# leejaehot/GaussianGrasper

Hardware: AMD Instinct MI355X
Metric: rendered views/sec (fwd+bwd) at 1M Gaussians, 1600x1200, 32-ch feature (higher is better)
Workload: dtype f32; 1 GPU; BASELINE config 4 per-GPU share: 1000000 Gaussians, 1600x1200, SH deg 4 rgb + 32-ch feature + depth + normal images per view (nerfstudio plugin route: the timed callable is FusedGaussianSplattingModel.get_outputs(camera) of gaussiangrasper_amd.plugin (the class train.sh loads, on stub.py's stand-ins for nerfstudio's base model and Cameras) — one fused rasterize operator per view), fwd+bwd, 8 views; route=plugin, deterministic_backward=False, python_gc=gc.freeze() after the warm-up (bench.freeze_gc), view_pipeline=backward of view k beside forward of view k + 1 on two streams, num_gaussians=1000000, feature_dim=32, n_visible=992125, parallelism=view-parallel x1, replicated Gaussians, grad_allreduce_bytes=472000000, grad_allreduce=per parameter, overlapped with the last view's backward

## Files before the change

### gaussiangrasper_amd/csrc/binning.hip

```cpp
#include "scan.h"

__device__ __forceinline__ int64_t dev_count(int64_t n, const int64_t *__restrict__ n_dev) {
    if (n_dev) {
        const int64_t d = *n_dev;
        if (d < n) n = d;
    }
    return n;
}

#define RS_THREADS 256
#define RS_WAVES (RS_THREADS / GG_WAVE)
#ifndef GG_RS_BIG
#define GG_RS_BIG 16
#endif
static inline int rs_items(int64_t n) { return n >= (int64_t)4096 * 1024 ? GG_RS_BIG : 4; }

__global__ __launch_bounds__(256) void count_kernel(int N, const int32_t *__restrict__ nth,
                                                    unsigned long long *__restrict__ out) {
    __shared__ unsigned long long part[4];
    unsigned long long acc = 0;
    for (int i = blockIdx.x * blockDim.x + threadIdx.x; i < N; i += gridDim.x * blockDim.x)
        acc += (unsigned long long)(uint32_t)nth[i];
    for (int off = 32; off > 0; off >>= 1) acc += __shfl_down(acc, off, 64);
    if ((threadIdx.x & 63) == 0) part[threadIdx.x >> 6] = acc;
// ... 127 lines not shown
        int64_t idx = wbase + (int64_t)it * GG_WAVE + lane;
        bool valid = idx < n;
        uint32_t d = (key[it] >> shift) & mask;
        uint64_t peers = __ballot(valid);
#pragma unroll
        for (int b = 0; b < 8; ++b) {
            if (b < nbits) {
                bool bit = (d >> b) & 1u;
                uint64_t m = __ballot(bit);
                peers &= bit ? m : ~m;
            }
        }
        uint32_t cnt = (uint32_t)__popcll(peers);
        uint32_t before = (uint32_t)__popcll(peers & lt_mask);
        uint32_t old = 0u;
        if (valid && before == 0) old = atomicAdd(&whist[wave][d], cnt);
        old = __shfl(old, (int)__builtin_ctzll(peers | (1ull << 63)), 64);
        rank[it] = old + before;
    }
    __syncthreads();
    __shared__ uint32_t lstart[256];
    __shared__ uint32_t skey[RS_TILE], sval[RS_TILE];
    {
        uint32_t run = 0;
        for (int w = 0; w < RS_WAVES; ++w) {
            uint32_t c = whist[w][tid];
            whist[w][tid] = run;
            run += c;
        }
        uint32_t incl = run;
        for (int off = 1; off < 64; off <<= 1) {
            uint32_t u = __shfl_up(incl, off, 64);
            if (lane >= off) incl += u;
        }
        if (lane == 63) wsum[wave] = incl;
        __syncthreads();
        uint32_t wpre = 0;
        for (int w = 0; w < wave; ++w) wpre += wsum[w];
        lstart[tid] = wpre + incl - run;
    }
    __syncthreads();
#pragma unroll
    for (int it = 0; it < RS_ITEMS; ++it) {
        int64_t idx = wbase + (int64_t)it * GG_WAVE + lane;
        if (idx < n) {
            uint32_t d = (key[it] >> shift) & mask;
            uint32_t lp = lstart[d] + whist[wave][d] + rank[it];
            skey[lp] = key[it];
            sval[lp] = val[it];
        }
    }
    __syncthreads();
    const int64_t left = n - (int64_t)blockIdx.x * RS_TILE;
    const int count = (int)(left < RS_TILE ? left : RS_TILE);
    for (int jj = tid; jj < count; jj += RS_THREADS) {
        const uint32_t k = skey[jj];
        const uint32_t d = (k >> shift) & mask;
        const uint32_t dst = digit_base[d] + ((uint32_t)jj - lstart[d]);
        keys_out[dst] = k;
        vals_out[dst] = sval[jj];
    }
}


typedef unsigned long long u64;
#define DB_BLOCKS 64
#define DB_THREADS 1024
#define DB_CAP 512
#define DB_MAX_BUCKETS 32768
static inline int db_buckets(int N) {
    int nb = 256;
    while (nb < DB_MAX_BUCKETS && nb * 64 < N) nb <<= 1;
    return nb;
}
struct DbRange {
    uint32_t kmin;
    u64 mul;
};
struct DbParts {
    const uint32_t *lo, *hi;
    int n;
};
__device__ __forceinline__ DbRange db_range_of(const DbParts mm, int nb, uint32_t *s_mm ) {
    const int tid = threadIdx.x;
    if (tid < 64) {
        uint32_t lo = 0xFFFFFFFFu, hi = 0u;
        for (int i = tid; i < mm.n; i += 64) {
            lo = min(lo, mm.lo[i]);
            hi = max(hi, mm.hi[i]);
        }
        for (int off = 32; off > 0; off >>= 1) {
            lo = min(lo, (uint32_t)__shfl_xor((int)lo, off, 64));
            hi = max(hi, (uint32_t)__shfl_xor((int)hi, off, 64));
        }
        if (tid == 0) { s_mm[0] = lo; s_mm[1] = hi; }
    }
    __syncthreads();
    DbRange r;
    const uint32_t lo = s_mm[0], hi = s_mm[1];
    r.kmin = lo;
    const u64 span = hi >= lo ? (u64)(hi - lo) + 1ull : 1ull;
    r.mul = (((u64)nb) << 32) / span;
    return r;
}
__device__ __forceinline__ uint32_t db_bucket(const DbRange r, uint32_t key, int nb) {
    if (key == 0xFFFFFFFFu) return (uint32_t)nb;
    return min((uint32_t)(((u64)(key - r.kmin) * r.mul) >> 32), (uint32_t)(nb - 1));
}
__global__ __launch_bounds__(256) void db_range_kernel(int N, DepthSrc dsrc, uint32_t *__restrict__ mm) {
    __shared__ uint32_t s_lo[4], s_hi[4];
    uint32_t lo = 0xFFFFFFFFu, hi = 0u;
    const int stride = 256 * gridDim.x;
    for (int i = blockIdx.x * 256 + threadIdx.x; i < N; i += 4 * stride) {
        uint32_t k[4];
#pragma unroll
        for (int u = 0; u < 4; ++u) k[u] = (i + u * stride < N) ? depth_key(dsrc, i + u * stride) : 0xFFFFFFFFu;
#pragma unroll
        for (int u = 0; u < 4; ++u)
            if (k[u] != 0xFFFFFFFFu) { lo = min(lo, k[u]); hi = max(hi, k[u]); }
    }
    for (int off = 32; off > 0; off >>= 1) {
        lo = min(lo, (uint32_t)__shfl_xor((int)lo, off, 64));
        hi = max(hi, (uint32_t)__shfl_xor((int)hi, off, 64));
    }
    if ((threadIdx.x & 63) == 0) { s_lo[threadIdx.x >> 6] = lo; s_hi[threadIdx.x >> 6] = hi; }
    __syncthreads();
    if (threadIdx.x == 0) {
        mm[blockIdx.x] = min(min(s_lo[0], s_lo[1]), min(s_lo[2], s_lo[3]));
        mm[gridDim.x + blockIdx.x] = max(max(s_hi[0], s_hi[1]), max(s_hi[2], s_hi[3]));
    }
}
#define DB_BOX_MAX 1023
struct DbGeom {
    const float *xys;
    int tiles_x, tiles_y;
};
__device__ __forceinline__ void db_box(const DbGeom g, const DepthSrc d, int i, uint32_t &cnt, uint32_t &box) {
    const int rad = d.radii[i];
    cnt = 0u;
    box = 1u << 20;
    if (rad > 0) {
        int x0, y0, x1, y1;
        gg_tile_bbox(g.xys[2 * (size_t)i], g.xys[2 * (size_t)i + 1], (float)rad, g.tiles_x, g.tiles_y, x0, y0, x1, y1);
        const int bw = x1 - x0;
        if (bw > 0 && y1 > y0) {
            cnt = (uint32_t)(bw * (y1 - y0));
            box = (uint32_t)x0 | ((uint32_t)y0 << 10) | ((uint32_t)bw << 20);
        }
    }
}
template <bool SCATTER>
__global__ __launch_bounds__(DB_THREADS) void db_walk_kernel(int N, int nb, DepthSrc dsrc, DbGeom geom,
                                                             const DbParts mm, uint32_t *__restrict__ G,
                                                             const uint32_t *__restrict__ start, uint4 *__restrict__ recs,
                                                             int32_t *__restrict__ zero = nullptr, int nzero = 0) {
    for (int i = blockIdx.x * DB_THREADS + threadIdx.x; i < nzero; i += DB_BLOCKS * DB_THREADS) zero[i] = 0;
    extern __shared__ uint32_t s_hist[];
    uint32_t *s_mm = s_hist + nb + 1;
    const DbRange r = db_range_of(mm, nb, s_mm);
    const int per = (N + DB_BLOCKS - 1) / DB_BLOCKS;
    const int lo = blockIdx.x * per, hi = min(N, lo + per);
    uint32_t *row = G + (size_t)blockIdx.x * (nb + 1);
    for (int b = threadIdx.x; b <= nb; b += DB_THREADS) s_hist[b] = SCATTER ? start[b] + row[b] : 0u;
    __syncthreads();
    for (int i = lo + threadIdx.x; i < hi; i += 4 * DB_THREADS) {
        uint32_t k[4], cnt[4], box[4];
#pragma unroll
        for (int u = 0; u < 4; ++u) {
            const int iu = i + u * DB_THREADS;
            k[u] = iu < hi ? depth_key(dsrc, iu) : 0u;
            cnt[u] = box[u] = 0u;
            if (SCATTER && iu < hi) db_box(geom, dsrc, iu, cnt[u], box[u]);
        }
#pragma unroll
        for (int u = 0; u < 4; ++u) {
            if (i + u * DB_THREADS < hi) {
                const uint32_t pos = atomicAdd(&s_hist[db_bucket(r, k[u], nb)], 1u);
                if (SCATTER && k[u] != 0xFFFFFFFFu)
                    recs[pos] = make_uint4(k[u], (uint32_t)(i + u * DB_THREADS), cnt[u], box[u]);
            }
        }
    }
    if (!SCATTER) {
        __syncthreads();
        for (int b = threadIdx.x; b <= nb; b += DB_THREADS) row[b] = s_hist[b];
    }
}
__global__ __launch_bounds__(256) void db_prefix_kernel(int nb, uint32_t *__restrict__ G, uint32_t *__restrict__ total) {
    const int b = blockIdx.x * 256 + threadIdx.x;
    if (b > nb) return;
    uint32_t run = 0;
    uint32_t c[DB_BLOCKS];
#pragma unroll
    for (int k = 0; k < DB_BLOCKS; ++k) c[k] = G[(size_t)k * (nb + 1) + b];
#pragma unroll
    for (int k = 0; k < DB_BLOCKS; ++k) {
        G[(size_t)k * (nb + 1) + b] = run;
        run += c[k];
    }
    total[b] = run;
}
__global__ __launch_bounds__(1024) void db_scan_kernel(int n, uint32_t *__restrict__ v) {
    __shared__ uint32_t s_w[2][16];
    const int tid = threadIdx.x, lane = tid & 63, wave = tid >> 6;
    uint32_t carry = 0u;
    int round = 0;
    for (int base = 0; base < n; base += 4 * 4096) {
        uint32_t x[4][4];
#pragma unroll
        for (int q = 0; q < 4; ++q)
#pragma unroll
            for (int k = 0; k < 4; ++k) {
                const int i = base + 4096 * q + 4 * tid + k;
                x[q][k] = i < n ? v[i] : 0u;
            }
#pragma unroll
        for (int q = 0; q < 4; ++q, ++round) {
            if (base + 4096 * q >= n) break;
            const uint32_t mine = x[q][0] + x[q][1] + x[q][2] + x[q][3];
            uint32_t incl = mine;
#pragma unroll
            for (int off = 1; off < 64; off <<= 1) {
                const uint32_t t = __shfl_up(incl, off, 64);
                if (lane >= off) incl += t;
            }
            uint32_t *sw = s_w[round & 1];
            if (lane == 63) sw[wave] = incl;
            __syncthreads();
            uint32_t ex = carry + incl - mine, all = 0u;
#pragma unroll
            for (int w = 0; w < 16; ++w) {
                const uint32_t t = sw[w];
                if (w < wave) ex += t;
                all += t;
            }
            carry += all;
#pragma unroll
            for (int k = 0; k < 4; ++k) {
                const int i = base + 4096 * q + 4 * tid + k;
                if (i < n) v[i] = ex;
                ex += x[q][k];
            }
        }
    }
    if (tid == 0) v[n] = carry;
}

__device__ __forceinline__ void db_ce(u64 &a, u64 &b) {
    const bool sw = b < a;
    const u64 lo = sw ? b : a, hi = sw ? a : b;
    a = lo;
    b = hi;
}
__device__ __forceinline__ void db_bitonic64(u64 *buf, const int n) {
    constexpr int NB = 8, LNB = 3, THREADS = 64;
    const int tid = threadIdx.x & 63;
    int P = NB;
    while (P < n) P <<= 1;
    const u64 INF = ~0ull;
    for (int blk = tid; blk * NB < n; blk += THREADS) {
        u64 v[NB];
#pragma unroll
        for (int r = 0; r < NB; ++r) v[r] = (NB * blk + r < n) ? buf[NB * blk + r] : INF;
#pragma unroll
        for (int k = 2; k <= NB; k <<= 1) {
#pragma unroll
            for (int i = 0; i < NB / 2; ++i) {
                const int b2 = i / (k / 2), off = i % (k / 2);
                db_ce(v[b2 * k + off], v[b2 * k + k - 1 - off]);
            }
#pragma unroll
            for (int j = k >> 2; j >= 1; j >>= 1)
#pragma unroll
                for (int i = 0; i < NB / 2; ++i) {
                    const int lo = ((i & ~(j - 1)) << 1) | (i & (j - 1));
                    db_ce(v[lo], v[lo + j]);
                }
        }
#pragma unroll
        for (int r = 0; r < NB; ++r)
            if (NB * blk + r < n) buf[NB * blk + r] = v[r];
    }
    { __builtin_amdgcn_fence(__ATOMIC_ACQ_REL, "workgroup"); __builtin_amdgcn_wave_barrier(); }
    for (int k = 2 * NB, lk = LNB + 1; k <= P; k <<= 1, ++lk) {
        const int hk = k >> 1;
        for (int i = tid; i < (P >> 1); i += THREADS) {
            const int blk = i >> (lk - 1), off = i & (hk - 1);
            const int lo = blk * k + off, hi = blk * k + k - 1 - off;
            if (hi < n) {
                const u64 a = buf[lo], b = buf[hi];
                if (b < a) { buf[lo] = b; buf[hi] = a; }
            }
        }
        { __builtin_amdgcn_fence(__ATOMIC_ACQ_REL, "workgroup"); __builtin_amdgcn_wave_barrier(); }
        for (int j = k >> 2; j >= NB; j >>= 1) {
            for (int i = tid; i < (P >> 1); i += THREADS) {
                const int lo = ((i & ~(j - 1)) << 1) | (i & (j - 1)), hi = lo + j;
                if (hi < n) {
                    const u64 a = buf[lo], b = buf[hi];
                    if (b < a) { buf[lo] = b; buf[hi] = a; }
                }
            }
            { __builtin_amdgcn_fence(__ATOMIC_ACQ_REL, "workgroup"); __builtin_amdgcn_wave_barrier(); }
        }
        for (int blk = tid; blk * NB < n; blk += THREADS) {
            u64 v[NB];
#pragma unroll
            for (int r = 0; r < NB; ++r) v[r] = (NB * blk + r < n) ? buf[NB * blk + r] : INF;
#pragma unroll
// ... 90 lines not shown
            gid[r] = in ? xw[64 * r + lane] : 0u;
            cntv[r] = in ? xw[DB_RANK_CAP + 64 * r + lane] : 0u;
            boxv[r] = in ? xw[2 * DB_RANK_CAP + 64 * r + lane] : 0u;
        }
    } else if (n <= DB_CAP) {
#define DB_LIM(nv) int nv = n - lane; asm volatile("" : "+v"(nv))
        u64 key[DB_ITEMS];
        {
            DB_LIM(nv);
#pragma unroll
            for (int r = 0; r < DB_ITEMS; ++r) {
                const uint4 rc = (64 * r < nv) ? recs[s0 + 64 * r + lane] : make_uint4(~0u, ~0u, 0u, 0u);
                key[r] = ((u64)rc.x << 32) | rc.y;
            }
        }
        auto pass = [&](const int shift) {
#pragma unroll
            for (int k = 0; k < 4; ++k) hist[lane + 64 * k] = 0u;
            db_wsync();
            {
                DB_LIM(nv);
#pragma unroll
                for (int r = 0; r < DB_ITEMS; ++r)
                    if (64 * r < nv) atomicAdd(&hist[(uint32_t)(key[r] >> shift) & 255u], 1u);
            }
            db_wsync();
            uint32_t tot[4], mine = 0;
            bool constant = false;
#pragma unroll
            for (int k = 0; k < 4; ++k) {
                tot[k] = hist[4 * lane + k];
                constant = constant || tot[k] == (uint32_t)n;
                mine += tot[k];
            }
            if (__ballot(constant) != 0ull) {
                db_wsync();
                return;
            }
            uint32_t incl = mine;
#pragma unroll
            for (int off = 1; off < 64; off <<= 1) {
                const uint32_t u = __shfl_up(incl, off, 64);
                if (lane >= off) incl += u;
            }
            uint32_t ex = incl - mine;
#pragma unroll
            for (int k = 0; k < 4; ++k) {
                hist[4 * lane + k] = ex;
                ex += tot[k];
            }
            db_wsync();
            volatile uint32_t *wh = hist;
            DB_LIM(nv_s);
#pragma unroll
            for (int r = 0; r < DB_ITEMS; ++r) {
                if (64 * r < n) {
                    const bool valid = 64 * r < nv_s;
                    const uint32_t d = (uint32_t)(key[r] >> shift) & 255u;
                    uint64_t peers = __ballot(valid);
#pragma unroll
                    for (int bit = 0; bit < 8; ++bit) {
                        const bool on = (d >> bit) & 1u;
                        const uint64_t m = __ballot(on);
                        peers &= on ? m : ~m;
                    }
                    const uint32_t cnt = (uint32_t)__popcll(peers);
                    const uint32_t before = (uint32_t)__popcll(peers & lt_mask);
                    if (valid && before == 0) wh[d] = wh[d] + cnt;
                    db_wsync();
                    if (valid) buf[wh[d] - cnt + before] = key[r];
                    db_wsync();
                    __builtin_amdgcn_sched_barrier(0);
                }
            }
            {
                DB_LIM(nv);
#pragma unroll
                for (int r = 0; r < DB_ITEMS; ++r) key[r] = (64 * r < nv) ? buf[64 * r + lane] : ~0ull;
            }
            db_wsync();
        };
#pragma nounroll
        for (int round = 0; round < 2; ++round) {
#pragma nounroll
            for (int pb = round == 0 ? 4 : 0; pb < 8; ++pb) pass(8 * pb);
            if (round == 1) break;
            {
                DB_LIM(nv);
#pragma unroll
                for (int r = 0; r < DB_ITEMS; ++r)
                    if (64 * r < nv) buf[64 * r + lane] = key[r];
            }
            db_wsync();
            bool bad = false;
            {
                DB_LIM(nv);
#pragma unroll
                for (int r = 0; r < DB_ITEMS; ++r)
                    if (64 * r + 1 < nv) {
                        const u64 nx = buf[64 * r + lane + 1];
                        bad = bad || ((uint32_t)(nx >> 32) == (uint32_t)(key[r] >> 32) && (uint32_t)nx < (uint32_t)key[r]);
                    }
            }
            db_wsync();
            if (__ballot(bad) == 0ull) break;
        }
#undef DB_LIM
#pragma unroll
        for (int r = 0; r < DB_ITEMS; ++r) gid[r] = (uint32_t)key[r];
    } else {
        for (int i = lane; i < n; i += 64) {
            const uint4 rc = recs[s0 + i];
            pairs[s0 + i] = ((u64)rc.x << 32) | rc.y;
        }
        db_wsync();
        db_bitonic64(pairs + s0, n);
    }
    uint32_t carry = 0;
    for (int c0 = 0; c0 < n; c0 += DB_CAP) {
        if (n > DB_CAP) {
#pragma unroll
            for (int r = 0; r < DB_ITEMS; ++r) gid[r] = (c0 + 64 * r + lane < n) ? (uint32_t)pairs[s0 + c0 + 64 * r + lane] : 0u;
        }
#pragma unroll
        for (int r = 0; r < DB_ITEMS; ++r) {
            const int p = c0 + 64 * r + lane;
            if (c0 + 64 * r < n) {
                const bool valid = p < n;
                const uint32_t g = min(gid[r], (uint32_t)(N - 1));
                uint32_t c = cntv[r], bx = boxv[r];
                if (!carried) {
                    c = 0u;
                    bx = 1u << 20;
                    if (valid) db_box(geom, dsrc, (int)g, c, bx);
                }
                if (!valid) c = 0u;
                uint32_t incl = c;
#pragma unroll
                for (int off = 1; off < 64; off <<= 1) {
                    const uint32_t u = __shfl_up(incl, off, 64);
                    if (lane >= off) incl += u;
                }
                if (valid) {
                    order[s0 + p] = g;
                    einfo[s0 + p] = make_uint4(carry + incl - c, (uint32_t)b, bx, c);
                }
                carry += __shfl(incl, 63, 64);
            }
        }
    }
    if (lane == 0) bucket_sum[b] = carry;
}

__global__ __launch_bounds__(256) void emit_kernel(int N, const uint32_t *__restrict__ order,
                                                   const uint4 *__restrict__ einfo,
                                                   const uint32_t *__restrict__ bucket_base,
                                                   const uint32_t *__restrict__ visible, int tiles_x,
                                                   int64_t I, const int64_t *__restrict__ I_dev,
                                                   uint32_t *__restrict__ tkeys,
                                                   uint32_t *__restrict__ tvals) {
    __shared__ uint32_t s_rel[4][64];
    I = dev_count(I, I_dev);
    __shared__ int4 s_box[4][64];
    const int lane = threadIdx.x & 63, wave = threadIdx.x >> 6;
    const int r = blockIdx.x * blockDim.x + threadIdx.x;
    uint32_t g = 0, cnt = 0, off = 0;
    int x0 = 0, y0 = 0, bw = 1;
    if (r < N && (uint32_t)r < *visible) {
        g = min(order[r], (uint32_t)(N - 1));
        const uint4 e = einfo[r];
        off = e.x + bucket_base[e.y];
        x0 = (int)(e.z & 1023u);
        y0 = (int)((e.z >> 10) & 1023u);
        bw = max(1, (int)(e.z >> 20));
        cnt = e.w;
    }
    uint32_t incl = cnt;
    for (int d = 1; d < 64; d <<= 1) {
        uint32_t u = __shfl_up(incl, d, 64);
        if (lane >= d) incl += u;
    }
    const uint32_t total = __shfl(incl, 63, 64);
    const uint32_t base = __shfl(off, 0, 64);
    s_rel[wave][lane] = incl - cnt;
    s_box[wave][lane] = make_int4(x0, y0, bw, (int)g);
    __builtin_amdgcn_wave_barrier();
    const uint32_t *rel = s_rel[wave];
    for (uint32_t j = lane; j < total; j += 64) {
        int lo = 0;
#pragma unroll
        for (int step = 32; step > 0; step >>= 1)
            if (rel[lo + step] <= j) lo += step;
        const int4 b = s_box[wave][lo];
        const uint32_t k = j - rel[lo];
        const uint32_t row = k / (uint32_t)b.z;
        const int64_t cur = (int64_t)base + j;
        if (cur < I) {
            tkeys[cur] = (uint32_t)((b.y + (int)row) * tiles_x + b.x + (int)(k - row * (uint32_t)b.z));
            tvals[cur] = (uint32_t)b.w;
        }
    }
}

__global__ __launch_bounds__(256) void tile_bins_kernel(int64_t I, const int64_t *__restrict__ I_dev,
                                                        const uint32_t *__restrict__ tkeys_sorted,
                                                        uint32_t num_tiles,
                                                        int32_t *__restrict__ tile_bins,
                                                        int32_t *__restrict__ tile_out) {
    I = dev_count(I, I_dev);
    int64_t i = (int64_t)blockIdx.x * blockDim.x + threadIdx.x;
    if (i >= I) return;
    uint32_t cur = tkeys_sorted[i];
    if (tile_out) tile_out[i] = (int32_t)cur;
    const bool cur_ok = cur < num_tiles;
    if (i == 0 && cur_ok) tile_bins[2 * cur] = 0;
    if (i == I - 1 && cur_ok) tile_bins[2 * cur + 1] = (int32_t)I;
    if (i > 0) {
        uint32_t prev = tkeys_sorted[i - 1];
        if (prev != cur) {
            if (prev < num_tiles) tile_bins[2 * prev + 1] = (int32_t)i;
            if (cur_ok) tile_bins[2 * cur] = (int32_t)i;
        }
    }
}

static int radix_nblocks(int64_t n) {
    const int64_t tile = (int64_t)RS_THREADS * rs_items(n);
    return (int)((n + tile - 1) / tile);
}

struct BinWs {
    uint32_t *order;
    uint4 *einfo;
    uint32_t *G;
    uint32_t *totals;
    uint32_t *tkeyA, *tkeyB, *tvalTmp;
    uint4 *recs;
    u64 *pairs;
    uint32_t *dbG;
    uint32_t *dbStart;
    uint32_t *dbBase;
    uint32_t *dbmm;
    size_t bytes;
};
static BinWs bin_ws_layout(void *ws, int N, int64_t I) {
    BinWs w;
    size_t off = 0;
    auto take = [&](size_t nbytes) {
        char *p = ws ? (char *)ws + off : nullptr;
        off += gg_align_up(nbytes, 256);
        return (uint32_t *)p;
    };
    size_t n = (size_t)(N > 0 ? N : 1), i = (size_t)(I > 0 ? I : 1);
    w.order = take(4 * n);
    w.einfo = (uint4 *)take(16 * n);
    int nb = max(radix_nblocks(N), radix_nblocks(I));
    w.G = take(4 * 256 * (size_t)(nb + 1));
    w.totals = take(4 * 256);
    w.tkeyA = take(4 * i);
    w.tkeyB = take(4 * i);
    w.tvalTmp = take(4 * i);
    const size_t nbk = (size_t)db_buckets(N);
    w.recs = (uint4 *)take(16 * n);
    w.pairs = (u64 *)take(8 * n);
    w.dbG = take(4 * DB_BLOCKS * (nbk + 1));
    w.dbStart = take(4 * (nbk + 2));
    w.dbBase = take(4 * (nbk + 1));
    w.dbmm = take(4 * 2 * 256);
    w.bytes = off;
    return w;
}
extern "C" size_t gg_bin_sort_workspace(int num_points, int64_t num_intersects) {
    return bin_ws_layout(nullptr, num_points, num_intersects).bytes;
}

static void radix_pass(int64_t n, const int64_t *n_dev, const uint32_t *kin, const uint32_t *vin,
                       uint32_t *kout, uint32_t *vout, int shift, uint32_t mask, BinWs &w, hipStream_t s,
                       DepthSrc dsrc = DepthSrc{nullptr, nullptr}) {
    int nb = radix_nblocks(n);
    if (rs_items(n) != 4)
        hipLaunchKernelGGL(radix_hist_kernel<GG_RS_BIG>, dim3(nb), dim3(RS_THREADS), 0, s, n, n_dev, kin, shift,
                           mask, nb, w.G, dsrc);
    else
        hipLaunchKernelGGL(radix_hist_kernel<4>, dim3(nb), dim3(RS_THREADS), 0, s, n, n_dev, kin, shift,
                           mask, nb, w.G, dsrc);
    hipLaunchKernelGGL(radix_colscan_kernel, dim3(256), dim3(256), 0, s, nb, w.G, w.totals);
    if (rs_items(n) != 4)
        hipLaunchKernelGGL(radix_scatter_kernel<GG_RS_BIG>, dim3(nb), dim3(RS_THREADS), 0, s, n, n_dev, kin, vin,
                           kout, vout, shift, mask, nb, w.G, w.totals, dsrc);
    else
        hipLaunchKernelGGL(radix_scatter_kernel<4>, dim3(nb), dim3(RS_THREADS), 0, s, n, n_dev, kin, vin,
                           kout, vout, shift, mask, nb, w.G, w.totals, dsrc);
}

static int bin_sort_impl(int N, int64_t I, const int64_t *I_dev, const float *xys, const float *depths,
                         const int32_t *radii, const int32_t *num_tiles_hit, int tiles_x, int tiles_y,
                         int32_t *gaussian_ids_sorted, int32_t *tile_bins, int32_t *isect_tile_sorted,
                         void *ws, size_t ws_bytes, gg_stream_t stream, const uint32_t *range_lo = nullptr,
                         const uint32_t *range_hi = nullptr, int range_parts = 0) {
    GG_REQUIRE(N >= 0 && I >= 0, "negative size");
    GG_REQUIRE(tiles_x > 0 && tiles_y > 0, "empty tile grid");
    GG_REQUIRE(tiles_x <= DB_BOX_MAX && tiles_y <= DB_BOX_MAX, "tile grid beyond 1023 x 1023 (images beyond 16 368 pixels a side)");
    GG_REQUIRE(I < (int64_t)1 << 31, "num_intersects must fit int32 (tile_bins are int32)");
    GG_REQUIRE(tile_bins != nullptr, "null tile_bins");
    hipStream_t s = (hipStream_t)stream;
    const int T = tiles_x * tiles_y;
    if (N == 0 || I == 0) {
        if (gg_fill_async(tile_bins, 0, sizeof(int32_t) * 2 * (size_t)T, s) != hipSuccess) {
            gg_set_error("gg_bin_sort: memset failed");
            return GG_ERR_LAUNCH;
        }
        return GG_OK;
    }
    GG_REQUIRE(xys && depths && radii && num_tiles_hit && gaussian_ids_sorted, "null pointer");
    BinWs w = bin_ws_layout(ws, N, I);
    if (ws == nullptr || ws_bytes < w.bytes) {
        gg_set_error("gg_bin_sort: workspace too small (%zu < %zu)", ws_bytes, w.bytes);
        return GG_ERR_WORKSPACE;
    }
    gg_prof_begin(GG_K_BIN_SORT, s);
    const int nbk = db_buckets(N);
    const DepthSrc dsrc{depths, radii};
    const size_t walk_lds = sizeof(uint32_t) * ((size_t)nbk + 1 + 2);
    if (walk_lds > 64 * 1024) {
        (void)hipFuncSetAttribute((const void *)db_walk_kernel<false>, hipFuncAttributeMaxDynamicSharedMemorySize, (int)walk_lds);
        (void)hipFuncSetAttribute((const void *)db_walk_kernel<true>, hipFuncAttributeMaxDynamicSharedMemorySize, (int)walk_lds);
    }
    uint32_t *order = w.order;
    DbParts mm{w.dbmm, w.dbmm + 256, 256};
    if (range_lo && range_hi && range_parts > 0)
        mm = DbParts{range_lo, range_hi, range_parts};
    else
        hipLaunchKernelGGL(db_range_kernel, dim3(256), dim3(256), 0, s, N, dsrc, w.dbmm);
    const DbGeom geom{xys, tiles_x, tiles_y};
    hipLaunchKernelGGL(db_walk_kernel<false>, dim3(DB_BLOCKS), dim3(DB_THREADS), walk_lds, s, N, nbk, dsrc, geom, mm,
                       w.dbG, (const uint32_t *)nullptr, (uint4 *)nullptr, tile_bins, 2 * T);
    hipLaunchKernelGGL(db_prefix_kernel, dim3((nbk + 1 + 255) / 256), dim3(256), 0, s, nbk, w.dbG, w.dbStart);
    hipLaunchKernelGGL(db_scan_kernel, dim3(1), dim3(1024), 0, s, nbk, w.dbStart);
    hipLaunchKernelGGL(db_walk_kernel<true>, dim3(DB_BLOCKS), dim3(DB_THREADS), walk_lds, s, N, nbk, dsrc, geom, mm,
                       w.dbG, (const uint32_t *)w.dbStart, w.recs, (int32_t *)nullptr, 0);
    hipLaunchKernelGGL(db_sort_kernel, dim3((nbk + DB_WPB - 1) / DB_WPB), dim3(64 * DB_WPB), 0, s, N, nbk,
                       (const uint32_t *)w.dbStart, (const uint4 *)w.recs, w.pairs, dsrc, geom, order, w.einfo, w.dbBase);
    hipLaunchKernelGGL(db_scan_kernel, dim3(1), dim3(1024), 0, s, nbk, w.dbBase);
    int tile_bits = 1;
    while ((1 << tile_bits) < T) ++tile_bits;
    int passes = (tile_bits + 7) / 8;
    uint32_t *out_vals = (uint32_t *)gaussian_ids_sorted;
    uint32_t *kcur = w.tkeyA, *kalt = w.tkeyB;
    uint32_t *vcur = (passes % 2 == 0) ? out_vals : w.tvalTmp;
    uint32_t *valt = (passes % 2 == 0) ? w.tvalTmp : out_vals;
    if (!I_dev) {
        (void)gg_fill_async(kcur, 0xFF, sizeof(uint32_t) * (size_t)I, s);
        (void)gg_fill_async(vcur, 0, sizeof(uint32_t) * (size_t)I, s);
    }
    hipLaunchKernelGGL(emit_kernel, dim3((N + 255) / 256), dim3(256), 0, s, N, (const uint32_t *)order,
                       (const uint4 *)w.einfo, (const uint32_t *)w.dbBase, (const uint32_t *)(w.dbStart + nbk), tiles_x, I,
                       I_dev, kcur, vcur);
    const int per_pass = (tile_bits + passes - 1) / passes;
    for (int pass = 0; pass < passes; ++pass) {
        int bits = min(per_pass, tile_bits - per_pass * pass);
        radix_pass(I, I_dev, kcur, vcur, kalt, valt, per_pass * pass, (1u << bits) - 1u, w, s);
        uint32_t *t = kcur; kcur = kalt; kalt = t;
        t = vcur; vcur = valt; valt = t;
    }
    hipLaunchKernelGGL(tile_bins_kernel, dim3((unsigned)((I + 255) / 256)), dim3(256), 0, s, I, I_dev, kcur,
                       (uint32_t)T, tile_bins, isect_tile_sorted);
    gg_prof_end(GG_K_BIN_SORT, s);
    GG_CHECK_LAUNCH();
    return GG_OK;
}

extern "C" int gg_bin_sort_status(int N, int64_t I, const void *ws, size_t ws_bytes, gg_stream_t stream) {
    GG_REQUIRE(N >= 0 && I >= 0, "negative size");
    (void)ws;
    (void)ws_bytes;
    if (hipStreamSynchronize((hipStream_t)stream) != hipSuccess) {
        gg_set_error("gg_bin_sort_status: stream synchronisation failed");
        return GG_ERR_LAUNCH;
    }
    return GG_OK;
}

extern "C" int gg_bin_sort(int N, int64_t I, const float *xys, const float *depths,
                           const int32_t *radii, const int32_t *num_tiles_hit, int tiles_x,
                           int tiles_y, int32_t *gaussian_ids_sorted, int32_t *tile_bins,
                           int32_t *isect_tile_sorted, void *ws, size_t ws_bytes,
                           gg_stream_t stream) {
    return bin_sort_impl(N, I, nullptr, xys, depths, radii, num_tiles_hit, tiles_x, tiles_y,
                         gaussian_ids_sorted, tile_bins, isect_tile_sorted, ws, ws_bytes, stream);
}

extern "C" int gg_bin_sort_dev(int N, int64_t capacity, const int64_t *num_intersects_dev,
                               const float *xys, const float *depths, const int32_t *radii,
                               const int32_t *num_tiles_hit, int tiles_x, int tiles_y,
                               int32_t *gaussian_ids_sorted, int32_t *tile_bins,
                               int32_t *isect_tile_sorted, void *ws, size_t ws_bytes,
                               gg_stream_t stream) {
    GG_REQUIRE(num_intersects_dev != nullptr, "null num_intersects_dev");
    GG_REQUIRE(capacity >= 1, "capacity < 1");
    return bin_sort_impl(N, capacity, num_intersects_dev, xys, depths, radii, num_tiles_hit, tiles_x,
                         tiles_y, gaussian_ids_sorted, tile_bins, isect_tile_sorted, ws, ws_bytes, stream);
}

extern "C" int gg_bin_sort_dev_ex(int N, int64_t capacity, const int64_t *num_intersects_dev,
                                  const float *xys, const float *depths, const int32_t *radii,
                                  const int32_t *num_tiles_hit, int tiles_x, int tiles_y,
                                  int32_t *gaussian_ids_sorted, int32_t *tile_bins,
                                  int32_t *isect_tile_sorted, void *ws, size_t ws_bytes,
                                  const uint32_t *depth_bits_min, const uint32_t *depth_bits_max, int range_parts,
                                  gg_stream_t stream) {
    GG_REQUIRE(num_intersects_dev != nullptr, "null num_intersects_dev");
    GG_REQUIRE(capacity >= 1, "capacity < 1");
    GG_REQUIRE(range_parts == 0 || (depth_bits_min && depth_bits_max && range_parts > 0), "range parts without arrays");
    return bin_sort_impl(N, capacity, num_intersects_dev, xys, depths, radii, num_tiles_hit, tiles_x,
                         tiles_y, gaussian_ids_sorted, tile_bins, isect_tile_sorted, ws, ws_bytes, stream,
                         depth_bits_min, depth_bits_max, range_parts);
}

size_t gg_sort_pairs_workspace(int64_t n) {
    const size_t i = (size_t)(n > 0 ? n : 1);
    return gg_align_up(4 * i, 256) * 2 + gg_align_up(4 * 256 * (size_t)(radix_nblocks(n) + 1), 256) +
           gg_align_up(4 * 256, 256);
}
int gg_sort_pairs(int64_t n, uint32_t *keys, uint32_t *vals, int bits, void *ws, size_t ws_bytes, hipStream_t s) {
    if (n <= 0) return GG_OK;
    if (ws == nullptr || ws_bytes < gg_sort_pairs_workspace(n)) return GG_ERR_WORKSPACE;
    char *p = (char *)ws;
    const size_t i = (size_t)n;
    uint32_t *kalt = (uint32_t *)p;
    p += gg_align_up(4 * i, 256);
    uint32_t *valt = (uint32_t *)p;
    p += gg_align_up(4 * i, 256);
    BinWs w;
    w.G = (uint32_t *)p;
    p += gg_align_up(4 * 256 * (size_t)(radix_nblocks(n) + 1), 256);
    w.totals = (uint32_t *)p;
    uint32_t *kc = keys, *vc = vals, *ka = kalt, *va = valt;
    const int passes = (bits + 7) / 8;
    for (int pass = 0; pass < passes; ++pass) {
        const int b = min(8, bits - 8 * pass);
        radix_pass(n, nullptr, kc, vc, ka, va, 8 * pass, (1u << b) - 1u, w, s);
        uint32_t *t = kc; kc = ka; ka = t;
        t = vc; vc = va; va = t;
    }
    if (kc != keys) {
        if (hipMemcpyAsync(keys, kc, 4 * i, hipMemcpyDeviceToDevice, s) != hipSuccess) return GG_ERR_LAUNCH;
        if (hipMemcpyAsync(vals, vc, 4 * i, hipMemcpyDeviceToDevice, s) != hipSuccess) return GG_ERR_LAUNCH;
    }
    return GG_OK;
}
```

Baseline: 630.3 views/s.

## Replace tile-key radix sort with two-level row/column counting scatter

Replaces the emit-then-radix-sort of per-tile intersection keys with a stable two-stage counting scatter. Depth-sorted Gaussians are first bucketed by tile row using per-segment difference histograms, then each row is split into chunks and bucketed by tile column, writing gaussian ids and tile bins directly. This avoids materialising the full key/value arrays and the multiple radix passes, at the cost of six new kernels, LDS atomics with wave-level match_any aggregation, and a single-block-per-row column scan that may serialise on rows with many chunks. Order within a tile must stay depth-sorted, which relies on the per-segment offsets preserving input order.

```diff
diff --git a/gaussiangrasper_amd/csrc/binning.hip b/gaussiangrasper_amd/csrc/binning.hip
--- a/gaussiangrasper_amd/csrc/binning.hip
+++ b/gaussiangrasper_amd/csrc/binning.hip
@@ -303,9 +303,7 @@
 template <bool SCATTER>
 __global__ __launch_bounds__(DB_THREADS) void db_walk_kernel(int N, int nb, DepthSrc dsrc, DbGeom geom,
                                                              const DbParts mm, uint32_t *__restrict__ G,
-                                                             const uint32_t *__restrict__ start, uint4 *__restrict__ recs,
-                                                             int32_t *__restrict__ zero = nullptr, int nzero = 0) {
-    for (int i = blockIdx.x * DB_THREADS + threadIdx.x; i < nzero; i += DB_BLOCKS * DB_THREADS) zero[i] = 0;
+                                                             const uint32_t *__restrict__ start, uint4 *__restrict__ recs) {
     extern __shared__ uint32_t s_hist[];
     uint32_t *s_mm = s_hist + nb + 1;
     const DbRange r = db_range_of(mm, nb, s_mm);
@@ -702,75 +700,344 @@
     if (lane == 0) bucket_sum[b] = carry;
 }
 
-__global__ __launch_bounds__(256) void emit_kernel(int N, const uint32_t *__restrict__ order,
-                                                   const uint4 *__restrict__ einfo,
-                                                   const uint32_t *__restrict__ bucket_base,
-                                                   const uint32_t *__restrict__ visible, int tiles_x,
-                                                   int64_t I, const int64_t *__restrict__ I_dev,
-                                                   uint32_t *__restrict__ tkeys,
-                                                   uint32_t *__restrict__ tvals) {
-    __shared__ uint32_t s_rel[4][64];
+#define RW_SEG 256
+#define CW_CHUNK 512
+#define BW_WAVES 4
+#define BW_GRID 1024
+
+struct RowSpan {
+    int x0, y0, bw, h, wl;
+};
+__device__ __forceinline__ RowSpan row_span(const uint4 e, const uint32_t *__restrict__ bucket_base, int64_t I,
+                                            bool full) {
+    RowSpan s;
+    s.x0 = (int)(e.z & 1023u);
+    s.y0 = (int)((e.z >> 10) & 1023u);
+    s.bw = max(1, (int)(e.z >> 20));
+    s.h = (int)e.w / s.bw;
+    s.wl = s.bw;
+    if (!full) {
+        const int64_t avail = I - ((int64_t)e.x + bucket_base[e.y]);
+        if (avail <= 0) {
+            s.h = 0;
+        } else if (avail < (int64_t)e.w) {
+            s.h = (int)((avail + s.bw - 1) / s.bw);
+            s.wl = (int)(avail - (int64_t)(s.h - 1) * s.bw);
+        }
+    }
+    return s;
+}
+__device__ __forceinline__ uint32_t wave_incl(uint32_t v) {
+    const int lane = threadIdx.x & 63;
+#pragma unroll
+    for (int off = 1; off < 64; off <<= 1) {
+        const uint32_t t = __shfl_up(v, off, 64);
+        if (lane >= off) v += t;
+    }
+    return v;
+}
+__device__ __forceinline__ uint64_t match_any(uint32_t d, int nbits, uint64_t peers) {
+#pragma unroll
+    for (int b = 0; b < 10; ++b) {
+        if (b < nbits) {
+            const bool bit = (d >> b) & 1u;
+            const uint64_t m = __ballot(bit);
+            peers &= bit ? m : ~m;
+        }
+    }
+    return peers;
+}
+__device__ __forceinline__ int expand_src(const uint32_t *rel, uint32_t j) {
+    int lo = 0;
+#pragma unroll
+    for (int step = 32; step > 0; step >>= 1)
+        if (rel[lo + step] <= j) lo += step;
+    return lo;
+}
+
+__global__ __launch_bounds__(64 * BW_WAVES) void row_hist_kernel(int nseg, const uint4 *__restrict__ einfo,
+                                                                 const uint32_t *__restrict__ bucket_base, int nb,
+                                                                 const uint32_t *__restrict__ visible, int64_t I,
+                                                                 const int64_t *__restrict__ I_dev, int tiles_y,
+                                                                 uint32_t *__restrict__ G) {
+    extern __shared__ uint32_t s_dyn[];
+    const int lane = threadIdx.x & 63, wave = threadIdx.x >> 6;
+    const int seg = blockIdx.x * BW_WAVES + wave;
+    if (seg >= nseg) return;
     I = dev_count(I, I_dev);
-    __shared__ int4 s_box[4][64];
+    const bool full = (int64_t)bucket_base[nb] <= I;
+    const int V = (int)*visible, r0 = seg * RW_SEG;
+    uint32_t *dc = s_dyn + (size_t)wave * 2 * (tiles_y + 1), *dw = dc + tiles_y + 1;
+    for (int y = lane; y <= tiles_y; y += 64) dc[y] = dw[y] = 0u;
+    uint4 e[RW_SEG / 64];
+#pragma unroll
+    for (int k = 0; k < RW_SEG / 64; ++k) {
+        const int r = r0 + 64 * k + lane;
+        e[k] = r < V ? einfo[r] : make_uint4(0u, 0u, 1u << 20, 0u);
+    }
+    db_wsync();
+#pragma unroll
+    for (int k = 0; k < RW_SEG / 64; ++k) {
+        const RowSpan s = row_span(e[k], bucket_base, I, full);
+        if (s.h > 0) {
+            atomicAdd(&dc[s.y0], 1u);
+            atomicAdd(&dc[s.y0 + s.h], ~0u);
+            atomicAdd(&dw[s.y0], (uint32_t)s.bw);
+            if (s.wl != s.bw) atomicAdd(&dw[s.y0 + s.h - 1], (uint32_t)(s.wl - s.bw));
+            atomicAdd(&dw[s.y0 + s.h], (uint32_t)-s.wl);
+        }
+    }
+    db_wsync();
+    uint32_t cc = 0u, cw = 0u;
+    for (int y0 = 0; y0 < tiles_y; y0 += 64) {
+        const int y = y0 + lane;
+        const uint32_t a = wave_incl(y < tiles_y ? dc[y] : 0u) + cc, b = wave_incl(y < tiles_y ? dw[y] : 0u) + cw;
+        if (y < tiles_y) {
+            G[(size_t)y * nseg + seg] = a;
+            G[(size_t)(tiles_y + y) * nseg + seg] = b;
+        }
+        cc = __shfl(a, 63, 64);
+        cw = __shfl(b, 63, 64);
+    }
+}
+
+__global__ __launch_bounds__(64 * BW_WAVES) void row_scatter_kernel(
+    int nseg, const uint32_t *__restrict__ order, const uint4 *__restrict__ einfo,
+    const uint32_t *__restrict__ bucket_base, int nb, const uint32_t *__restrict__ visible, int64_t I,
+    const int64_t *__restrict__ I_dev, int N, int tiles_y, const uint32_t *__restrict__ G,
+    const uint32_t *__restrict__ totals, uint2 *__restrict__ rows) {
+    extern __shared__ uint32_t s_dyn[];
+    __shared__ uint4 s_g[BW_WAVES][RW_SEG];
+    __shared__ uint32_t s_rel[BW_WAVES][64];
     const int lane = threadIdx.x & 63, wave = threadIdx.x >> 6;
-    const int r = blockIdx.x * blockDim.x + threadIdx.x;
-    uint32_t g = 0, cnt = 0, off = 0;
-    int x0 = 0, y0 = 0, bw = 1;
-    if (r < N && (uint32_t)r < *visible) {
-        g = min(order[r], (uint32_t)(N - 1));
-        const uint4 e = einfo[r];
-        off = e.x + bucket_base[e.y];
-        x0 = (int)(e.z & 1023u);
-        y0 = (int)((e.z >> 10) & 1023u);
-        bw = max(1, (int)(e.z >> 20));
-        cnt = e.w;
-    }
-    uint32_t incl = cnt;
-    for (int d = 1; d < 64; d <<= 1) {
-        uint32_t u = __shfl_up(incl, d, 64);
-        if (lane >= d) incl += u;
-    }
-    const uint32_t total = __shfl(incl, 63, 64);
-    const uint32_t base = __shfl(off, 0, 64);
-    s_rel[wave][lane] = incl - cnt;
-    s_box[wave][lane] = make_int4(x0, y0, bw, (int)g);
-    __builtin_amdgcn_wave_barrier();
-    const uint32_t *rel = s_rel[wave];
-    for (uint32_t j = lane; j < total; j += 64) {
-        int lo = 0;
-#pragma unroll
-        for (int step = 32; step > 0; step >>= 1)
-            if (rel[lo + step] <= j) lo += step;
-        const int4 b = s_box[wave][lo];
-        const uint32_t k = j - rel[lo];
-        const uint32_t row = k / (uint32_t)b.z;
-        const int64_t cur = (int64_t)base + j;
-        if (cur < I) {
-            tkeys[cur] = (uint32_t)((b.y + (int)row) * tiles_x + b.x + (int)(k - row * (uint32_t)b.z));
-            tvals[cur] = (uint32_t)b.w;
-        }
-    }
-}
-
-__global__ __launch_bounds__(256) void tile_bins_kernel(int64_t I, const int64_t *__restrict__ I_dev,
-                                                        const uint32_t *__restrict__ tkeys_sorted,
-                                                        uint32_t num_tiles,
-                                                        int32_t *__restrict__ tile_bins,
-                                                        int32_t *__restrict__ tile_out) {
+    const int seg = blockIdx.x * BW_WAVES + wave;
+    if (seg >= nseg) return;
     I = dev_count(I, I_dev);
-    int64_t i = (int64_t)blockIdx.x * blockDim.x + threadIdx.x;
-    if (i >= I) return;
-    uint32_t cur = tkeys_sorted[i];
-    if (tile_out) tile_out[i] = (int32_t)cur;
-    const bool cur_ok = cur < num_tiles;
-    if (i == 0 && cur_ok) tile_bins[2 * cur] = 0;
-    if (i == I - 1 && cur_ok) tile_bins[2 * cur + 1] = (int32_t)I;
-    if (i > 0) {
-        uint32_t prev = tkeys_sorted[i - 1];
-        if (prev != cur) {
-            if (prev < num_tiles) tile_bins[2 * prev + 1] = (int32_t)i;
-            if (cur_ok) tile_bins[2 * cur] = (int32_t)i;
-        }
+    const bool full = (int64_t)bucket_base[nb] <= I;
+    const int V = (int)*visible, r0 = seg * RW_SEG;
+    if (r0 >= V) return;
+    const int m = min(RW_SEG, V - r0);
+    uint4 e[RW_SEG / 64];
+    uint32_t id[RW_SEG / 64];
+#pragma unroll
+    for (int k = 0; k < RW_SEG / 64; ++k) {
+        const bool in = 64 * k + lane < m;
+        e[k] = in ? einfo[r0 + 64 * k + lane] : make_uint4(0u, 0u, 1u << 20, 0u);
+        id[k] = in ? min(order[r0 + 64 * k + lane], (uint32_t)(N - 1)) : 0u;
+    }
+    uint32_t *cur = s_dyn + (size_t)wave * tiles_y;
+    {
+        uint32_t carry = 0u;
+        for (int y0 = 0; y0 < tiles_y; y0 += 64) {
+            const int y = y0 + lane;
+            const uint32_t v = y < tiles_y ? totals[y] : 0u, incl = wave_incl(v);
+            if (y < tiles_y) cur[y] = carry + incl - v + G[(size_t)y * nseg + seg];
+            carry += __shfl(incl, 63, 64);
+        }
+    }
+#pragma unroll
+    for (int k = 0; k < RW_SEG / 64; ++k) {
+        const RowSpan s = row_span(e[k], bucket_base, I, full);
+        s_g[wave][64 * k + lane] = make_uint4(id[k], (uint32_t)s.x0 | ((uint32_t)s.y0 << 10),
+                                              (uint32_t)s.bw | ((uint32_t)s.wl << 10) | ((uint32_t)s.h << 20), 0u);
+    }
+    db_wsync();
+    const int nbits = 32 - __builtin_clz((uint32_t)max(tiles_y - 1, 1));
+    const uint64_t lt_mask = (lane == 0) ? 0ull : (~0ull >> (64 - lane));
+    uint32_t *rel = s_rel[wave];
+    for (int k0 = 0; k0 < m; k0 += 64) {
+        const uint4 g = s_g[wave][k0 + lane];
+        const uint32_t h = k0 + lane < m ? g.z >> 20 : 0u;
+        const uint32_t incl = wave_incl(h), total = __shfl(incl, 63, 64);
+        rel[lane] = incl - h;
+        db_wsync();
+        for (uint32_t j0 = 0; j0 < total; j0 += 64) {
+            const uint32_t j = j0 + lane;
+            const bool valid = j < total;
+            const int src = expand_src(rel, valid ? j : 0u);
+            const uint4 b = s_g[wave][k0 + src];
+            const uint32_t row = j - rel[src], hb = b.z >> 20;
+            const uint32_t y = ((b.y >> 10) & 1023u) + row;
+            const uint32_t wdt = row + 1 == hb ? (b.z >> 10) & 1023u : b.z & 1023u;
+            const uint64_t peers = match_any(y, nbits, __ballot(valid));
+            const uint32_t cnt = (uint32_t)__popcll(peers), before = (uint32_t)__popcll(peers & lt_mask);
+            uint32_t old = 0u;
+            if (valid && before == 0) old = atomicAdd(&cur[y], cnt);
+            old = __shfl(old, (int)__builtin_ctzll(peers | (1ull << 63)), 64);
+            if (valid) rows[old + before] = make_uint2(b.x, (b.y & 1023u) | (wdt << 10));
+        }
+        db_wsync();
+    }
+}
+
+__device__ __forceinline__ bool col_chunk(int gid, const uint32_t *__restrict__ totals, int tiles_y, int &y, int &c,
+                                          uint32_t &first, uint32_t &len) {
+    const int lane = threadIdx.x & 63;
+    uint32_t rcarry = 0u, ccarry = 0u;
+    for (int y0 = 0; y0 < tiles_y; y0 += 64) {
+        const int yy = y0 + lane;
+        const uint32_t v = yy < tiles_y ? totals[yy] : 0u, nc = (v + CW_CHUNK - 1) / CW_CHUNK;
+        const uint32_t ri = wave_incl(v), ci = wave_incl(nc);
+        const uint32_t rex = rcarry + ri - v, cex = ccarry + ci - nc;
+        const uint64_t hit = __ballot(yy < tiles_y && (uint32_t)gid >= cex && (uint32_t)gid < cex + nc);
+        if (hit) {
+            const int src = (int)__builtin_ctzll(hit);
+            y = y0 + src;
+            first = __shfl(rex, src, 64);
+            len = __shfl(v, src, 64);
+            c = gid - (int)__shfl(cex, src, 64);
+            return true;
+        }
+        rcarry += __shfl(ri, 63, 64);
+        ccarry += __shfl(ci, 63, 64);
+    }
+    return false;
+}
+
+__global__ __launch_bounds__(64 * BW_WAVES) void col_hist_kernel(int nchunk, const uint32_t *__restrict__ totals,
+                                                                 int tiles_x, int tiles_y, const uint2 *__restrict__ rows,
+                                                                 uint32_t *__restrict__ Gc) {
+    extern __shared__ uint32_t s_dyn[];
+    const int lane = threadIdx.x & 63, wave = threadIdx.x >> 6;
+    const int gid = blockIdx.x * BW_WAVES + wave;
+    if (gid >= nchunk) return;
+    int y, c;
+    uint32_t first, len;
+    if (!col_chunk(gid, totals, tiles_y, y, c, first, len)) return;
+    const uint32_t e0 = first + (uint32_t)c * CW_CHUNK, m = min((uint32_t)CW_CHUNK, len - (uint32_t)c * CW_CHUNK);
+    uint32_t *d = s_dyn + (size_t)wave * (tiles_x + 1);
+    for (int x = lane; x <= tiles_x; x += 64) d[x] = 0u;
+    uint32_t xw[CW_CHUNK / 64];
+#pragma unroll
+    for (int k = 0; k < CW_CHUNK / 64; ++k) xw[k] = 64 * k + lane < (int)m ? rows[e0 + 64 * k + lane].y : 0u;
+    db_wsync();
+#pragma unroll
+    for (int k = 0; k < CW_CHUNK / 64; ++k) {
+        const uint32_t w = xw[k] >> 10, x0 = xw[k] & 1023u;
+        if (w) {
+            atomicAdd(&d[x0], 1u);
+            atomicAdd(&d[x0 + w], ~0u);
+        }
+    }
+    db_wsync();
+    uint32_t carry = 0u;
+    for (int x0 = 0; x0 < tiles_x; x0 += 64) {
+        const int x = x0 + lane;
+        const uint32_t a = wave_incl(x < tiles_x ? d[x] : 0u) + carry;
+        if (x < tiles_x) Gc[(size_t)gid * tiles_x + x] = a;
+        carry = __shfl(a, 63, 64);
+    }
+}
+
+__global__ __launch_bounds__(1024) void col_scan_kernel(int64_t I, const int64_t *__restrict__ I_dev,
+                                                        const uint32_t *__restrict__ totals, int tiles_x, int tiles_y,
+                                                        uint32_t *__restrict__ Gc, int32_t *__restrict__ tile_bins,
+                                                        int32_t *__restrict__ ids, int32_t *__restrict__ isect) {
+    __shared__ uint32_t s_r[3], s_w[16];
+    const int y = blockIdx.x, tid = threadIdx.x, lane = tid & 63, wave = tid >> 6;
+    uint32_t cb = 0u, tb = 0u, ta = 0u;
+    if (tid < tiles_y) {
+        ta = totals[tiles_y + tid];
+        if (tid < y) {
+            cb = (totals[tid] + CW_CHUNK - 1) / CW_CHUNK;
+            tb = ta;
+        }
+    }
+    if (tid < 3) s_r[tid] = 0u;
+#pragma unroll
+    for (int off = 32; off > 0; off >>= 1) {
+        cb += __shfl_xor(cb, off, 64);
+        tb += __shfl_xor(tb, off, 64);
+        ta += __shfl_xor(ta, off, 64);
+    }
+    __syncthreads();
+    if (lane == 0 && cb) atomicAdd(&s_r[0], cb);
+    if (lane == 0 && tb) atomicAdd(&s_r[1], tb);
+    if (lane == 0 && ta) atomicAdd(&s_r[2], ta);
+    __syncthreads();
+    const uint32_t cs = s_r[0], row_start = s_r[1], total = s_r[2];
+    const int nch = (int)((totals[y] + CW_CHUNK - 1) / CW_CHUNK);
+    uint32_t run = 0u;
+    if (tid < tiles_x) {
+        uint32_t *col = Gc + (size_t)cs * tiles_x + tid;
+        for (int c0 = 0; c0 < nch; c0 += 8) {
+            uint32_t v[8];
+#pragma unroll
+            for (int k = 0; k < 8; ++k) v[k] = c0 + k < nch ? col[(size_t)(c0 + k) * tiles_x] : 0u;
+#pragma unroll
+            for (int k = 0; k < 8; ++k)
+                if (c0 + k < nch) {
+                    col[(size_t)(c0 + k) * tiles_x] = run;
+                    run += v[k];
+                }
+        }
+    }
+    const uint32_t incl = wave_incl(run);
+    if (lane == 63) s_w[wave] = incl;
+    __syncthreads();
+    uint32_t ex = incl - run;
+    for (int w = 0; w < wave; ++w) ex += s_w[w];
+    if (tid < tiles_x) {
+        const uint32_t st = row_start + ex;
+        const size_t t = (size_t)y * tiles_x + tid;
+        tile_bins[2 * t] = run ? (int32_t)st : 0;
+        tile_bins[2 * t + 1] = run ? (int32_t)(st + run) : 0;
+    }
+    I = dev_count(I, I_dev);
+    for (int64_t i = (int64_t)total + (int64_t)y * 1024 + tid; i < I; i += (int64_t)gridDim.x * 1024) {
+        ids[i] = 0;
+        if (isect) isect[i] = -1;
+    }
+}
+
+__global__ __launch_bounds__(64 * BW_WAVES) void col_scatter_kernel(
+    int nchunk, const uint32_t *__restrict__ totals, int tiles_x, int tiles_y, const uint2 *__restrict__ rows,
+    const uint32_t *__restrict__ Gc, const int32_t *__restrict__ tile_bins, int32_t *__restrict__ ids,
+    int32_t *__restrict__ isect) {
+    extern __shared__ uint32_t s_dyn[];
+    __shared__ uint2 s_e[BW_WAVES][CW_CHUNK];
+    __shared__ uint32_t s_rel[BW_WAVES][64];
+    const int lane = threadIdx.x & 63, wave = threadIdx.x >> 6;
+    const int gid = blockIdx.x * BW_WAVES + wave;
+    if (gid >= nchunk) return;
+    int y, c;
+    uint32_t first, len;
+    if (!col_chunk(gid, totals, tiles_y, y, c, first, len)) return;
+    const uint32_t e0 = first + (uint32_t)c * CW_CHUNK, m = min((uint32_t)CW_CHUNK, len - (uint32_t)c * CW_CHUNK);
+    uint2 *se = s_e[wave];
+#pragma unroll
+    for (int k = 0; k < CW_CHUNK / 64; ++k)
+        if (64 * k + lane < (int)m) se[64 * k + lane] = rows[e0 + 64 * k + lane];
+    uint32_t *cur = s_dyn + (size_t)wave * tiles_x;
+    for (int x = lane; x < tiles_x; x += 64)
+        cur[x] = Gc[(size_t)gid * tiles_x + x] + (uint32_t)tile_bins[2 * ((size_t)y * tiles_x + x)];
+    db_wsync();
+    const int nbits = 32 - __builtin_clz((uint32_t)max(tiles_x - 1, 1));
+    const uint64_t lt_mask = (lane == 0) ? 0ull : (~0ull >> (64 - lane));
+    const uint32_t tile0 = (uint32_t)y * tiles_x;
+    uint32_t *rel = s_rel[wave];
+    for (uint32_t k0 = 0; k0 < m; k0 += 64) {
+        const uint32_t w = k0 + lane < m ? se[k0 + lane].y >> 10 : 0u;
+        const uint32_t incl = wave_incl(w), total = __shfl(incl, 63, 64);
+        rel[lane] = incl - w;
+        db_wsync();
+        for (uint32_t j0 = 0; j0 < total; j0 += 64) {
+            const uint32_t j = j0 + lane;
+            const bool valid = j < total;
+            const int src = expand_src(rel, valid ? j : 0u);
+            const uint2 b = se[k0 + src];
+            const uint32_t x = (b.y & 1023u) + (j - rel[src]);
+            const uint64_t peers = match_any(x, nbits, __ballot(valid));
+            const uint32_t cnt = (uint32_t)__popcll(peers), before = (uint32_t)__popcll(peers & lt_mask);
+            uint32_t old = 0u;
+            if (valid && before == 0) old = atomicAdd(&cur[x], cnt);
+            old = __shfl(old, (int)__builtin_ctzll(peers | (1ull << 63)), 64);
+            if (valid) {
+                ids[old + before] = (int32_t)b.x;
+                if (isect) isect[old + before] = (int32_t)(tile0 + x);
+            }
+        }
+        db_wsync();
     }
 }
 
@@ -784,15 +1051,20 @@
     uint4 *einfo;
     uint32_t *G;
     uint32_t *totals;
-    uint32_t *tkeyA, *tkeyB, *tvalTmp;
     uint4 *recs;
     u64 *pairs;
     uint32_t *dbG;
     uint32_t *dbStart;
     uint32_t *dbBase;
     uint32_t *dbmm;
+    uint32_t *rowG;
+    uint32_t *rowTot;
+    uint2 *rows;
+    uint32_t *colG;
     size_t bytes;
 };
+static int row_segments(int N) { return (N + RW_SEG - 1) / RW_SEG; }
+static int col_chunks(int64_t I, int tiles_y) { return (int)((I + CW_CHUNK - 1) / CW_CHUNK) + tiles_y; }
 static BinWs bin_ws_layout(void *ws, int N, int64_t I) {
     BinWs w;
     size_t off = 0;
@@ -804,12 +1076,7 @@
     size_t n = (size_t)(N > 0 ? N : 1), i = (size_t)(I > 0 ? I : 1);
     w.order = take(4 * n);
     w.einfo = (uint4 *)take(16 * n);
-    int nb = max(radix_nblocks(N), radix_nblocks(I));
-    w.G = take(4 * 256 * (size_t)(nb + 1));
-    w.totals = take(4 * 256);
-    w.tkeyA = take(4 * i);
-    w.tkeyB = take(4 * i);
-    w.tvalTmp = take(4 * i);
+    w.G = w.totals = nullptr;
     const size_t nbk = (size_t)db_buckets(N);
     w.recs = (uint4 *)take(16 * n);
     w.pairs = (u64 *)take(8 * n);
@@ -817,6 +1084,10 @@
     w.dbStart = take(4 * (nbk + 2));
     w.dbBase = take(4 * (nbk + 1));
     w.dbmm = take(4 * 2 * 256);
+    w.rowG = take(4 * 2 * BW_GRID * (size_t)row_segments((int)n));
+    w.rowTot = take(4 * 2 * BW_GRID);
+    w.rows = (uint2 *)take(8 * i);
+    w.colG = take(4 * BW_GRID * (size_t)col_chunks((int64_t)i, BW_GRID));
     w.bytes = off;
     return w;
 }
@@ -884,37 +1155,31 @@
         hipLaunchKernelGGL(db_range_kernel, dim3(256), dim3(256), 0, s, N, dsrc, w.dbmm);
     const DbGeom geom{xys, tiles_x, tiles_y};
     hipLaunchKernelGGL(db_walk_kernel<false>, dim3(DB_BLOCKS), dim3(DB_THREADS), walk_lds, s, N, nbk, dsrc, geom, mm,
-                       w.dbG, (const uint32_t *)nullptr, (uint4 *)nullptr, tile_bins, 2 * T);
+                       w.dbG, (const uint32_t *)nullptr, (uint4 *)nullptr);
     hipLaunchKernelGGL(db_prefix_kernel, dim3((nbk + 1 + 255) / 256), dim3(256), 0, s, nbk, w.dbG, w.dbStart);
     hipLaunchKernelGGL(db_scan_kernel, dim3(1), dim3(1024), 0, s, nbk, w.dbStart);
     hipLaunchKernelGGL(db_walk_kernel<true>, dim3(DB_BLOCKS), dim3(DB_THREADS), walk_lds, s, N, nbk, dsrc, geom, mm,
-                       w.dbG, (const uint32_t *)w.dbStart, w.recs, (int32_t *)nullptr, 0);
+                       w.dbG, (const uint32_t *)w.dbStart, w.recs);
     hipLaunchKernelGGL(db_sort_kernel, dim3((nbk + DB_WPB - 1) / DB_WPB), dim3(64 * DB_WPB), 0, s, N, nbk,
                        (const uint32_t *)w.dbStart, (const uint4 *)w.recs, w.pairs, dsrc, geom, order, w.einfo, w.dbBase);
     hipLaunchKernelGGL(db_scan_kernel, dim3(1), dim3(1024), 0, s, nbk, w.dbBase);
-    int tile_bits = 1;
-    while ((1 << tile_bits) < T) ++tile_bits;
-    int passes = (tile_bits + 7) / 8;
-    uint32_t *out_vals = (uint32_t *)gaussian_ids_sorted;
-    uint32_t *kcur = w.tkeyA, *kalt = w.tkeyB;
-    uint32_t *vcur = (passes % 2 == 0) ? out_vals : w.tvalTmp;
-    uint32_t *valt = (passes % 2 == 0) ? w.tvalTmp : out_vals;
-    if (!I_dev) {
-        (void)gg_fill_async(kcur, 0xFF, sizeof(uint32_t) * (size_t)I, s);
-        (void)gg_fill_async(vcur, 0, sizeof(uint32_t) * (size_t)I, s);
-    }
-    hipLaunchKernelGGL(emit_kernel, dim3((N + 255) / 256), dim3(256), 0, s, N, (const uint32_t *)order,
-                       (const uint4 *)w.einfo, (const uint32_t *)w.dbBase, (const uint32_t *)(w.dbStart + nbk), tiles_x, I,
-                       I_dev, kcur, vcur);
-    const int per_pass = (tile_bits + passes - 1) / passes;
-    for (int pass = 0; pass < passes; ++pass) {
-        int bits = min(per_pass, tile_bits - per_pass * pass);
-        radix_pass(I, I_dev, kcur, vcur, kalt, valt, per_pass * pass, (1u << bits) - 1u, w, s);
-        uint32_t *t = kcur; kcur = kalt; kalt = t;
-        t = vcur; vcur = valt; valt = t;
-    }
-    hipLaunchKernelGGL(tile_bins_kernel, dim3((unsigned)((I + 255) / 256)), dim3(256), 0, s, I, I_dev, kcur,
-                       (uint32_t)T, tile_bins, isect_tile_sorted);
+    const uint32_t *visible = w.dbStart + nbk;
+    const int nseg = row_segments(N), nchunk = col_chunks(I, tiles_y);
+    const dim3 rgrid((nseg + BW_WAVES - 1) / BW_WAVES), cgrid((nchunk + BW_WAVES - 1) / BW_WAVES), wgb(64 * BW_WAVES);
+    const size_t lds_y = 4 * BW_WAVES * (size_t)(tiles_y + 1), lds_x = 4 * BW_WAVES * (size_t)(tiles_x + 1);
+    hipLaunchKernelGGL(row_hist_kernel, rgrid, wgb, 2 * lds_y, s, nseg, (const uint4 *)w.einfo, (const uint32_t *)w.dbBase, nbk,
+                       visible, I, I_dev, tiles_y, w.rowG);
+    hipLaunchKernelGGL(radix_colscan_kernel, dim3(2 * tiles_y), dim3(256), 0, s, nseg, w.rowG, w.rowTot);
+    hipLaunchKernelGGL(row_scatter_kernel, rgrid, wgb, lds_y, s, nseg, (const uint32_t *)order, (const uint4 *)w.einfo,
+                       (const uint32_t *)w.dbBase, nbk, visible, I, I_dev, N, tiles_y, (const uint32_t *)w.rowG,
+                       (const uint32_t *)w.rowTot, w.rows);
+    hipLaunchKernelGGL(col_hist_kernel, cgrid, wgb, lds_x, s, nchunk, (const uint32_t *)w.rowTot, tiles_x, tiles_y,
+                       (const uint2 *)w.rows, w.colG);
+    hipLaunchKernelGGL(col_scan_kernel, dim3(tiles_y), dim3(1024), 0, s, I, I_dev, (const uint32_t *)w.rowTot, tiles_x,
+                       tiles_y, w.colG, tile_bins, gaussian_ids_sorted, isect_tile_sorted);
+    hipLaunchKernelGGL(col_scatter_kernel, cgrid, wgb, lds_x, s, nchunk, (const uint32_t *)w.rowTot, tiles_x, tiles_y,
+                       (const uint2 *)w.rows, (const uint32_t *)w.colG, (const int32_t *)tile_bins, gaussian_ids_sorted,
+                       isect_tile_sorted);
     gg_prof_end(GG_K_BIN_SORT, s);
     GG_CHECK_LAUNCH();
     return GG_OK;
```

Measured after the change: 638.3 views/s (median of 6 runs). +1.3%, better.
